# duanyiqun/DiffusionDepth

Hardware: AMD Instinct MI355X
Metric: depth-maps/sec (20-step DDIM, KITTI 352x1216 f16r, B=4 maps per GPU per step; depth RMSE vs the reference's CPU path <= 1e-3 on this workload AND at KITTI's depth range 0-80 m: see cpu_baseline.rmse_gate) (higher is better)
Workload: dtype f16 (f16 MFMA operands, fp32 accumulation; refined mode: f16-pair weights in conv1 / conv4 / conv3(cond), block-scaled int16 hand-over of y3 and conv3(cond)); 1 GPU; kitti 352x1216 image -> latent 16x176x608, cond 256x176x608, Res head denoiser (mmbev_res50 config), T=20, encoder+loop+decoder, inputs resident in HBM; global_batch=4, parallelism=dp1 (independent images, no collective), ranks_seen=1, streams=2, graph=True, variant=res

## Files before the change

### diffusiondepth_amd/csrc/dd_api.cpp

```cpp
#include "dd_api_internal.h"
#include <cstdlib>

namespace ddapi {
thread_local std::string g_create_error;
}


extern "C" {

const char* dd_version(void) { return "ddepth 0.1 gfx950 (hip, mfma bf16/f16/f32 implicit-GEMM conv3x3+GN+ReLU, hipGraph DDIM loop)"; }

const char* dd_last_error(dd_handle_t h) { return h ? h->err.c_str() : g_create_error.c_str(); }

int dd_create(dd_handle_t* out, int device, int variant) {
  if (!out) { g_create_error = "dd_create: out is NULL"; return DD_ERR_INVALID_ARG; }
  *out = nullptr;
  if (variant != DD_VARIANT_RES && variant != DD_VARIANT_SWIN) { g_create_error = "dd_create: unknown variant"; return DD_ERR_INVALID_ARG; }
  int n = 0;
  hipError_t e = hipGetDeviceCount(&n);
  if (e != hipSuccess || n <= 0) {
    g_create_error = std::string("dd_create: no HIP device available (") + (e != hipSuccess ? hipGetErrorString(e) : "count = 0") +
                     "); this library has no CPU fallback";
    return DD_ERR_HIP;
  }
// ... 94 lines not shown
    h->bf16_pure = value != 0;
  }
  else if (k == "naive_wgrad") h->naive_wgrad = value != 0;
  else if (k == "lane_probe") h->lane_probe = value != 0;
  else if (k == "x3_grad_fp32") h->x3_grad_fp32 = value != 0;
  else if (k == "keep_trajectory") h->keep_traj = value != 0;
  else if (k == "use_trajectory") h->use_traj = value;
  else if (k == "adjoint_tiled") h->adjoint_tiled = value != 0;
  else if (k == "streams") h->n_streams = value < 1 ? 1 : (int)value;
  else if (k == "keep_activations_mb") h->keep_act_mb = value < 0 ? 0 : value;
  else if (k == "big_tiles") {
    if (value < -1 || value > 1) return h->fail(DD_ERR_INVALID_ARG, "dd_set_option: big_tiles must be -1 (automatic), 0 or 1");
    if (h->big_tiles != (int)value) { DD_HIP(hipDeviceSynchronize()); h->plans.clear(); h->last_once_plan = nullptr; }
    h->big_tiles = (int)value;
  }
  else if (k == "thin_slots") {
    if (value < 1 || value > 4096) return h->fail(DD_ERR_INVALID_ARG, "dd_set_option: thin_slots must be in [1, 4096]");
    if (h->thin_slots != (int)value) { DD_HIP(hipDeviceSynchronize()); h->plans.clear(); h->last_once_plan = nullptr; }
    h->thin_slots = (int)value;
  }
  else if (k == "one_buffer") {
    if (value < 0 || value > 2) return h->fail(DD_ERR_INVALID_ARG, "dd_set_option: one_buffer must be 0, 1 or 2");
    if (h->one_buffer != (int)value) { DD_HIP(hipDeviceSynchronize()); h->plans.clear(); h->last_once_plan = nullptr; }
    h->one_buffer = (int)value;
  }
  else if (k == "cond_direct") {
    if (value < 0 || value > 1) return h->fail(DD_ERR_INVALID_ARG, "dd_set_option: cond_direct must be 0 or 1");
    h->cond_direct = (int)value;
  }
  else if (k == "cond_split") {
    if (value < 0 || value > 1) return h->fail(DD_ERR_INVALID_ARG, "dd_set_option: cond_split must be 0 or 1");
    h->cond_split = (int)value;
  }
  else if (k == "thin_stream") {
    if (value < 0 || value > 1) return h->fail(DD_ERR_INVALID_ARG, "dd_set_option: thin_stream must be 0 or 1");
    if (h->thin_stream != (int)value) {
      DD_HIP(hipDeviceSynchronize());
      h->plans.clear(); h->last_once_plan = nullptr;
    }
    h->thin_stream = (int)value;
  }
  else if (k == "f16r_wide" || k == "f16r_p4" || k == "f16r_c1") {
    if (value < 0 || value > 1) return h->fail(DD_ERR_INVALID_ARG, "dd_set_option: " + k + " must be 0 or 1");
    int& opt = k == "f16r_wide" ? h->f16r_wide : k == "f16r_c1" ? h->f16r_c1 : h->f16r_p4;
    if (opt != (int)value) { DD_HIP(hipDeviceSynchronize()); h->plans.clear(); h->last_once_plan = nullptr; }
    opt = (int)value;
  }
  else if (k == "phase_prof_buffer") h->prof_buf = reinterpret_cast<unsigned long long*>((uintptr_t)value);
  else if (k == "phase_prof_layer") h->prof_layer = (int)value;
  else if (k == "layer_timing") {
    drain_layer_events(h);
    h->layer_timing = value != 0;
    for (int i = 0; i < dd_handle_s::N_LAYER_SLOTS; ++i) { h->layer_ms[i] = 0; h->layer_cnt[i] = 0; }
  } else return h->fail(DD_ERR_INVALID_ARG, "dd_set_option: unknown key '" + k + "'");
  return DD_OK;
}

int dd_get_counter(dd_handle_t h, const char* key, int64_t* value) {
  if (!h || !key || !value) return DD_ERR_INVALID_ARG;
  const std::string k(key);
  if (k == "graph_launches") *value = h->n_graph_launches;
  else if (k == "graph_default") *value = h->graph_off_by_env ? 0 : 1;
  else if (k == "eager_loops") *value = h->n_eager_loops;
  else if (k == "graph_capture_failures") *value = h->n_capture_failures;
  else if (k == "plans") *value = (int64_t)h->plans.size();
  else if (k == "neck_launches") *value = h->n_neck_launches;
  else if (k == "trajectory_ticket") *value = h->traj_serial;
  else if (k == "lane_calls") *value = h->n_lane_calls;
  else if (k == "lane_probe_retries") *value = h->n_lane_probe_retries;
  else if (k == "lane_overlap") *value = h->lane_overlap_seen;
  else if (k == "cond_split_ok") *value = (h->fpn_committed && h->fpn_split_ok ? 1 : 0) | (h->neck_committed && h->neck_split_ok ? 2 : 0);
  else if (k == "resident_slots") *value = h->resident_slots;
  else if (k == "trajectory_reuses") *value = h->n_traj_reuse;
  else return h->fail(DD_ERR_INVALID_ARG, "dd_get_counter: unknown key '" + k + "'");
  return DD_OK;
}

// ... 457 lines not shown
  }
  h->last_once_plan = pl;
  pl->traj_ticket = (h->keep_traj && precision != DD_PREC_NAIVE_FP32) ? ++h->traj_serial : 0;
  pl->traj_weights = h->weights_serial;
  if (h->debug_sync) DD_HIP(hipStreamSynchronize(s));
  return DD_OK;
}

int dd_add_noise(dd_handle_t h, const float* x0, const float* noise, const int64_t* t, float* out, int B, int C,
                 int lat_h, int lat_w, void* stream) {
  if (!h) return DD_ERR_INVALID_ARG;
  if (h->n_train <= 0) return h->fail(DD_ERR_STATE, "schedule not set (dd_set_schedule)");
  if (!x0 || !noise || !t || !out || B <= 0 || C <= 0 || lat_h <= 0 || lat_w <= 0)
    return h->fail(DD_ERR_INVALID_ARG, "dd_add_noise: null pointer or non-positive size");
  DD_HIP(hipSetDevice(h->device));
  DD_HIP(launch_add_noise(x0, noise, reinterpret_cast<const long long*>(t), h->d_acp.as<float>(), h->n_train, out, B,
                          (long long)C * lat_h * lat_w, reinterpret_cast<hipStream_t>(stream)));
  return DD_OK;
}

static int ensure_codec_tmp(dd_handle_t h, size_t bytes) {
  if (h->codec_tmp.bytes >= bytes) return DD_OK;
  DD_HIP(hipDeviceSynchronize());
  DD_HIP(h->codec_tmp.alloc(bytes));
  return DD_OK;
}

int dd_encode(dd_handle_t h, const float* depth, float* latent, int B, int H, int W, void* stream) {
  if (!h) return DD_ERR_INVALID_ARG;
  if (!h->codec_committed) return h->fail(DD_ERR_STATE, "depth_transform.* weights not committed");
  if (!depth || !latent || B <= 0 || H <= 0 || W <= 0) return h->fail(DD_ERR_INVALID_ARG, "dd_encode: null pointer or non-positive size");
  DD_HIP(hipSetDevice(h->device));
  const int lh = (H - 1) / 2 + 1, lw = (W - 1) / 2 + 1;
  int rc = ensure_codec_tmp(h, (size_t)B * lh * lw * LATENT_C * 4);
  if (rc) return rc;
  DD_HIP(launch_encode(h->codec, depth, h->codec_tmp.as<float>(), latent, B, H, W, reinterpret_cast<hipStream_t>(stream)));
  return DD_OK;
}

int dd_decode(dd_handle_t h, const float* latent, float* depth, int B, int lat_h, int lat_w, void* stream) {
  if (!h) return DD_ERR_INVALID_ARG;
  if (!h->codec_committed) return h->fail(DD_ERR_STATE, "depth_transform.* weights not committed");
  if (!latent || !depth || B <= 0 || lat_h <= 0 || lat_w <= 0) return h->fail(DD_ERR_INVALID_ARG, "dd_decode: null pointer or non-positive size");
  DD_HIP(hipSetDevice(h->device));
  int rc = ensure_codec_tmp(h, (size_t)B * (2 * lat_h) * (2 * lat_w) * LATENT_C * 4);
  if (rc) return rc;
  DD_HIP(launch_decode(h->codec, latent, h->codec_tmp.as<float>(), depth, B, lat_h, lat_w, reinterpret_cast<hipStream_t>(stream)));
  return DD_OK;
}

int dd_debug_fetch(dd_handle_t h, const char* name, float* out, int64_t numel, void* stream) {
  if (!h || !name || !out) return DD_ERR_INVALID_ARG;
  Plan* pl = h->last_once_plan;
  if (!pl) return h->fail(DD_ERR_STATE, "dd_debug_fetch: no dd_denoise_once call to inspect");
  const std::string n(name);
  const void* src = nullptr; int C = 0; int ek = store_kind(pl->ek);
  if (n == "y1") { src = pl->y1.p; C = HID_C; }
  else if (n == "y2") { src = pl->y2.p; C = COND_C; }
  else if (n == "y3") {
    src = pl->y3.p; C = HID_C;
    if (pl->ek == EK_F16R && pl->wide) return h->fail(DD_ERR_UNSUPPORTED, "dd_debug_fetch: y3 travels as scaled int16 in this plan (option f16r_wide = 1)");
  }
  else if (n == "y4") { src = pl->y4.p; C = LATENT_C; ek = EK_F32; }
  else return h->fail(DD_ERR_INVALID_ARG, "dd_debug_fetch: unknown tensor '" + n + "'");
  if (numel != (int64_t)pl->key.B * C * pl->key.h * pl->key.w) return h->fail(DD_ERR_INVALID_ARG, "dd_debug_fetch: numel mismatch");
  DD_HIP(launch_nhwc_to_nchw_f32(src, ek, out, pl->key.B, C, pl->key.h, pl->key.w, pl->key.prec != DD_PREC_NAIVE_FP32,
// ... 42 lines not shown
```

### diffusiondepth_amd/csrc/dd_api_internal.h

```cpp
#pragma once
#include "../../include/ddepth.h"
#include "dd_kernels.h"

#include <cmath>
#include <cstdio>
#include <cstring>
#include <map>
#include <memory>
#include <set>
#include <string>
#include <tuple>
#include <vector>

using namespace dd;

namespace ddapi {

extern thread_local std::string g_create_error;

struct DevBuf {
  void* p = nullptr;
  size_t bytes = 0;
  DevBuf() = default;
  DevBuf(const DevBuf&) = delete;
// ... 73 lines not shown
  int B, h, w, ch, cw, T, prec, hoist;
  int keep = 0;
  int lane = 0;
  int lanes = 1;
  bool operator<(const PlanKey& o) const {
    return std::tie(B, h, w, ch, cw, T, prec, hoist, keep, lane, lanes) < std::tie(o.B, o.h, o.w, o.ch, o.cw, o.T, o.prec, o.hoist, o.keep, o.lane, o.lanes);
  }
};

struct Plan {
  PlanKey key{};
  int ek = EK_F32;
  DevBuf x[2];
  std::shared_ptr<DevBuf> cond;
  const void* cond_alias = nullptr;
  const void* graph_cond = nullptr;
  void* cond_ptr() const { return cond_alias ? const_cast<void*>(cond_alias) : (cond ? cond->p : nullptr); }
  DevBuf y1, y2, y3, y4;
  DevBuf a1, f, a3, eps;
  DevBuf sa, sf;
  DevBuf bX, bA1, bF, bA3;
  DevBuf bSa, bSf;
  DevBuf xstash;
  int64_t traj_ticket = 0;
  int64_t traj_weights = -1;
  bool traj_consumed = false;
  DevBuf gA, gY;
  DevBuf dgb;
  DevBuf bcorr;
  DevBuf ttab, tt_scratch;
  int64_t ttab_weights = -1;
  DevBuf ccond;
  DevBuf ccond_raw;
  DevBuf ccond_scale;
  DevBuf y3_scale;
  bool wide = false, c1 = false, p4 = false;
  DevBuf stats;
  DevBuf c1c2;
  DevBuf tsteps;
  std::vector<long long> tsteps_host;
  size_t stats_bytes = 0;
  hipGraphExec_t exec = nullptr;
  bool capture_failed = false;
  uint64_t last_use = 0;
  ~Plan() { if (exec) (void)hipGraphExecDestroy(exec); }
  int slots = 1;
  size_t kept_bytes = 0;
  void* slot(const DevBuf& b, int step) const { return static_cast<char*>(b.p) + (slots > 1 ? (size_t)step * (b.bytes / slots) : 0); }
  double* stat_ptr(int step, int layer) const {
    return stats.as<double>() + ((size_t)(step * 4 + layer) * key.B) * STAT_SLOTS * STAT_STRIDE;
  }
};

struct FpnWork {
  int B = 0, ek = -1, pyr = 0, hs[FPN_LEVELS] = {0}, ws[FPN_LEVELS] = {0};
  DevBuf fin[FPN_LEVELS];
  DevBuf lat[FPN_LEVELS];
  DevBuf up[FPN_LEVELS - 1];
  DevBuf pooled[FPN_LEVELS - 1];
  bool neck = false;
  DevBuf nk_cat[FPN_LEVELS];
  DevBuf nk_out[FPN_LEVELS];
};


struct NeckConv { int layer; std::string name; int cout, cin, ks, level, kind, C, Ck; };
// ... 63 lines not shown
  int f16r_wide = 1;
  int f16r_c1 = 1;
  int f16r_p4 = 0;
  bool split_ok = true;
  DevBuf wmax;
  int resident_slots = 512;
  hipStream_t lane_stream[MAX_LANES] = {nullptr, nullptr, nullptr, nullptr};
  std::vector<hipEvent_t> probe_events;
  std::vector<hipStream_t> burnt_streams;
  int lane_probe = 1;
  int64_t n_lane_probe_retries = 0, lane_overlap_seen = -1;
  hipEvent_t lane_fork = nullptr, lane_done[MAX_LANES] = {nullptr, nullptr, nullptr, nullptr};
  int64_t n_lane_calls = 0;
  int active_lanes = 1;
  bool adjoint_tiled = true;
  int64_t traj_serial = 0, use_traj = 0, weights_serial = 0, n_traj_reuse = 0;
  int naive_wgrad = 0;
  int x3_grad_fp32 = 0;
  std::map<PlanKey, std::unique_ptr<Plan>> plans;
  DevBuf wgrad_ws[MAX_LANES];
  std::map<std::string, std::unique_ptr<DevBuf>> grads[MAX_LANES];
  std::map<std::tuple<int, int, int, int, int>, std::pair<std::shared_ptr<DevBuf>, uint64_t>> cond_bufs;
  bool neck_committed = false;
  DevBuf neck_w[12][NUM_WIMG], neck_b[12];
  int64_t n_neck_launches = 0;
  bool fpn_committed = false;
  int fpn_pyramid = PYR_DEFAULT;
  DevBuf fpn_lat_w[FPN_LEVELS][NUM_WIMG], fpn_lat_b[FPN_LEVELS];
  DevBuf fpn_up_w[FPN_LEVELS - 1][NUM_WIMG], fpn_up_b[FPN_LEVELS - 1];
  std::unique_ptr<FpnWork> fpn_work;
  std::shared_ptr<DevBuf> fpn_out;
  bool fpn_split_ok = false, neck_split_ok = false;
  int cond_direct = 1;
  int cond_split = 1;
  std::shared_ptr<DevBuf> fpn_cond;
  int fpn_cond_key[4] = {0, 0, 0, -1};
  uint64_t tick = 0;
  Plan* last_once_plan = nullptr;
  hipEvent_t ev0 = nullptr, ev1 = nullptr;
  bool ev_valid = false;
  hipStream_t cap_stream = nullptr;
  int64_t n_graph_launches = 0, n_eager_loops = 0, n_capture_failures = 0;
  static constexpr int N_LAYER_SLOTS = 72;
  double layer_ms[N_LAYER_SLOTS] = {0};
  int64_t layer_cnt[N_LAYER_SLOTS] = {0};
  std::vector<std::tuple<int, hipEvent_t, hipEvent_t>> pending_ev;

  int fail(int code, const std::string& m) { err = m; return code; }
};

#define DD_HIP(expr)                                                                              \
  do {                                                                                            \
    hipError_t _e = (expr);                                                                       \
    if (_e != hipSuccess)                                                                         \
      return h->fail(DD_ERR_HIP, std::string(#expr) + ": " + hipGetErrorString(_e));              \
  } while (0)

namespace ddapi {
struct WeightSpec { std::string name; int64_t numel; };

inline const char* const kConvNames[4] = {"model.noise_embedding.0", "model.noise_embedding.3", "model.pred.0", "model.pred.3"};
inline const char* const kGnNames[4] = {"model.noise_embedding.1", "model.noise_embedding.4", "model.pred.1", "model.pred.4"};
constexpr int kCins[4] = {LATENT_C, HID_C, COND_C, HID_C}, kCouts[4] = {HID_C, COND_C, HID_C, LATENT_C};

int weight_group(const std::string& name);
std::vector<WeightSpec> required_weights(int variant, int pyr = PYR_DEFAULT);
// ... 36 lines not shown
```

### diffusiondepth_amd/csrc/dd_api_plans.cpp

```cpp
#include "dd_api_internal.h"

namespace ddapi {

int check_common(dd_handle_t h, int B, int lh, int lw, int ch, int cw, bool need_schedule) {
  if (!h) return DD_ERR_INVALID_ARG;
  if (!h->committed) return h->fail(DD_ERR_STATE, "model.* weights not committed (call dd_set_weight for every key, then dd_commit_weights)");
  if (need_schedule && h->n_train <= 0) return h->fail(DD_ERR_STATE, "schedule not set (dd_set_schedule)");
  if (B <= 0 || lh <= 0 || lw <= 0) return h->fail(DD_ERR_INVALID_ARG, "B, lat_h, lat_w must be positive");
  if (h->variant == DD_VARIANT_RES && (ch != lh || cw != lw))
    return h->fail(DD_ERR_INVALID_ARG, "DD_VARIANT_RES needs cond_h,cond_w == lat_h,lat_w (reference ...res.py:340 adds them elementwise)");
  if (h->variant == DD_VARIANT_SWIN && (ch <= 0 || cw <= 0)) return h->fail(DD_ERR_INVALID_ARG, "cond_h, cond_w must be positive");
  if ((long long)B * lh * lw * COND_C >= (1LL << 31) * 4) return h->fail(DD_ERR_INVALID_ARG, "tensor too large");
  return DD_OK;
}

int lane_count(dd_handle_t h, int B, int precision) {
  int S = h->n_streams;
  if (S > B) S = B;
  if (S > dd_handle_s::MAX_LANES) S = dd_handle_s::MAX_LANES;
  if (precision == DD_PREC_NAIVE_FP32 || h->layer_timing || h->debug_sync || h->prof_buf || h->check_finite) S = 1;
  return S < 1 ? 1 : S;
}

int check_split(dd_handle_t h, int precision, const char* who) {
// ... 90 lines not shown
    }
    if (victim == h->plans.end()) break;
    if (h->last_once_plan == victim->second.get()) h->last_once_plan = nullptr;
    DD_HIP(hipDeviceSynchronize());
    h->plans.erase(victim);
  }
  std::unique_ptr<Plan> pl(new Plan());
  pl->key = key;
  const bool naive = key.prec == DD_PREC_NAIVE_FP32;
  pl->ek = naive ? EK_F32 : ek_of_precision(key.prec, h->bf16_pure);
  if (pl->ek == EK_F16R && !key.hoist)
    return h->fail(DD_ERR_UNSUPPORTED, "DD_PREC_F16R runs the hoisted forward-only plans: for the Swin / MPViT denoiser those exist with option swin_w5 = 1 "
                                       "(dd_denoise / dd_denoise_trace / dd_denoise_once); training plans: DD_PREC_F16");
  const size_t px = (size_t)key.B * key.h * key.w;
  const size_t es = ek_size(pl->ek);
  DD_HIP(pl->x[0].alloc(px * LATENT_C * 4));
  DD_HIP(pl->x[1].alloc(px * LATENT_C * 4));
  if (key.keep) DD_HIP(pl->xstash.alloc((size_t)(key.T > 0 ? key.T : 1) * px * LATENT_C * 4));
  const bool swin = h->variant == DD_VARIANT_SWIN;
  (void)swin;
  if (!(pl->ek == EK_F16R && !swin && key.hoist)) { int rc = get_cond_buf(h, key.B, key.h, key.w, key.prec, &pl->cond, key.lane); if (rc) return rc; }
  pl->slots = (key.keep == 2 && key.T > 0) ? key.T : 1;
  const size_t ns = (size_t)pl->slots;
  if (swin) {
    const size_t es_s = pl->ek == EK_F16R ? 4 : es;
    DD_HIP(pl->sa.alloc(ns * px * COND_C * es_s)); DD_HIP(pl->sf.alloc(ns * px * COND_C * es_s));
  }
  if (key.hoist)
  {
    const int th = conv_pack_geom2(conv3h_kid(h, key), pl->ek).th;
    DD_HIP(pl->ccond.alloc((size_t)key.B * ((key.h + th - 1) / th) * ((key.w + 31) / 32) * th * 32 * HID_C * 4));
    if (pl->ek == EK_F16R) {
      pl->wide = h->f16r_wide != 0; pl->c1 = h->f16r_c1 != 0; pl->p4 = h->f16r_p4 != 0;
      DD_HIP(pl->ccond_raw.alloc((size_t)key.B * ((key.h + 7) / 8) * ((key.w + 31) / 32) * 8 * 32 * HID_C * 4));
      if (pl->wide) DD_HIP(pl->ccond_scale.alloc((size_t)key.B * ((key.h + th - 1) / th) * ((key.w + 31) / 32) * 4 * 2 * (th / 4) * 4));
    }
  }
  if (key.hoist && swin) {
    const int T1 = key.T > 0 ? key.T : key.B;
    const int RH = key.h < SWIN_TT_AX ? key.h : SWIN_TT_AX, RW = key.w < SWIN_TT_AX ? key.w : SWIN_TT_AX;
    DD_HIP(pl->ttab.alloc((size_t)T1 * SWIN_TT_ROWS * HID_C * 4));
    DD_HIP(pl->tt_scratch.alloc((size_t)T1 * RH * RW * (2 * COND_C + HID_C) * 4));
    if (h->swin_w5) {
      DD_HIP(pl->bcorr.alloc((size_t)key.B * swin_ring_stride(key.h, key.w) * HID_C * 4));
      DD_HIP(hipMemsetAsync(pl->bcorr.p, 0, pl->bcorr.bytes, nullptr));
      DD_HIP(hipStreamSynchronize(nullptr));
    }
  }
  DD_HIP(pl->y1.alloc(ns * px * HID_C * es));
  DD_HIP(pl->y2.alloc(ns * px * COND_C * es));
  DD_HIP(pl->y3.alloc(ns * px * HID_C * es));
  if (pl->ek == EK_F16R && h->f16r_wide) DD_HIP(pl->y3_scale.alloc(ns * px * 4));
  DD_HIP(pl->y4.alloc(ns * px * LATENT_C * 4));
  if (key.keep == 2) pl->kept_bytes = pl->y1.bytes + pl->y2.bytes + pl->y3.bytes + pl->y3_scale.bytes + pl->y4.bytes + pl->sa.bytes + pl->sf.bytes;
  if (naive) {
    DD_HIP(pl->a1.alloc(px * HID_C * 4));
    DD_HIP(pl->f.alloc(px * COND_C * 4));
    DD_HIP(pl->a3.alloc(px * HID_C * 4));
    DD_HIP(pl->eps.alloc(px * LATENT_C * 4));
  }
  const int T = key.T > 0 ? key.T : 1;
  pl->stats_bytes = (size_t)(T + 1) * 4 * key.B * STAT_SLOTS * STAT_STRIDE * sizeof(double);
  DD_HIP(pl->stats.alloc(pl->stats_bytes));
  std::vector<float> c1c2((size_t)T * 2, 0.f);
  std::vector<long long> ts((size_t)T, 0);
  if (key.T > 0) {
    const int ratio = h->n_train / key.T;
    for (int k = 0; k < key.T; ++k) {
// ... 122 lines not shown
  const PlanKey& k = pl->key;
  const int B = k.B, hh = k.h, ww = k.w;
  auto L = h->L;
  DD_HIP(launch_naive_conv3x3(x_in, L[0].w_oihw.as<float>(), L[0].bias.as<float>(), pl->y1.as<float>(), B, hh, ww, LATENT_C, HID_C, s));
  DD_HIP(launch_naive_gn_stats(pl->y1.as<float>(), pl->stat_ptr(step, 0), B, hh, ww, HID_C, s));
  DD_HIP(launch_naive_gn_apply(pl->y1.as<float>(), pl->stat_ptr(step, 0), L[0].gamma.as<float>(), L[0].beta.as<float>(),
                               nullptr, nullptr, nullptr, 0, 0, pl->a1.as<float>(), B, hh, ww, HID_C, s));
  DD_HIP(launch_naive_conv3x3(pl->a1.as<float>(), L[1].w_oihw.as<float>(), L[1].bias.as<float>(), pl->y2.as<float>(), B, hh, ww, HID_C, COND_C, s));
  DD_HIP(launch_naive_gn_stats(pl->y2.as<float>(), pl->stat_ptr(step, 1), B, hh, ww, COND_C, s));
  DD_HIP(launch_naive_gn_apply(pl->y2.as<float>(), pl->stat_ptr(step, 1), L[1].gamma.as<float>(), L[1].beta.as<float>(),
                               static_cast<const float*>(pl->cond_ptr()), h->emb.as<float>(), tvec, t_base, t_bstride, pl->f.as<float>(), B, hh, ww, COND_C, s));
  DD_HIP(launch_naive_conv3x3(pl->f.as<float>(), L[2].w_oihw.as<float>(), L[2].bias.as<float>(), pl->y3.as<float>(), B, hh, ww, COND_C, HID_C, s));
  DD_HIP(launch_naive_gn_stats(pl->y3.as<float>(), pl->stat_ptr(step, 2), B, hh, ww, HID_C, s));
  DD_HIP(launch_naive_gn_apply(pl->y3.as<float>(), pl->stat_ptr(step, 2), L[2].gamma.as<float>(), L[2].beta.as<float>(),
                               nullptr, nullptr, nullptr, 0, 0, pl->a3.as<float>(), B, hh, ww, HID_C, s));
  DD_HIP(launch_naive_conv3x3(pl->a3.as<float>(), L[3].w_oihw.as<float>(), L[3].bias.as<float>(), pl->y4.as<float>(), B, hh, ww, HID_C, LATENT_C, s));
  DD_HIP(launch_naive_gn_stats(pl->y4.as<float>(), pl->stat_ptr(step, 3), B, hh, ww, LATENT_C, s));
  DD_HIP(launch_naive_gn_apply(pl->y4.as<float>(), pl->stat_ptr(step, 3), L[3].gamma.as<float>(), L[3].beta.as<float>(),
                               nullptr, nullptr, nullptr, 0, 0, pl->eps.as<float>(), B, hh, ww, LATENT_C, s));
  if (h->debug_sync) DD_HIP(hipStreamSynchronize(s));
  return DD_OK;
}

int enqueue_cond_conv(dd_handle_t h, Plan* pl, hipStream_t s, const float* nchw) {
  const PlanKey& k = pl->key;
  ConvParams p{};
  p.B = k.B; p.h = k.h; p.w = k.w;
  p.tiles_x = (k.w + 31) / 32;
  p.ablate = 0;
  if (pl->ek == EK_F16R) {
    p.tiles_y = (k.h + 7) / 8;
    p.in = nchw ? static_cast<const void*>(nchw) : pl->cond_ptr(); p.wpack = h->L[2].wpack2[WIMG_SPLIT].p; p.bias = h->zero_bias.as<float>();
    p.out = pl->ccond_raw.p;
    DD_HIP(launch_conv_igemm2(nchw ? CONV3C_NCHW : 8, EK_F16S, p, s));
    DD_HIP(launch_cadd_reformat(pl->ccond_raw.as<float>(), pl->ccond.p, pl->ccond_scale.as<float>(), k.B, k.h, k.w, plan_big_tiles(h, k) ? 1 : 0, pl->wide ? 2 : 1, s));
    return DD_OK;
  }
  const int kid = conv3c_kid(h, k);
  p.tiles_y = (k.h + conv_pack_geom2(kid, pl->ek).th - 1) / conv_pack_geom2(kid, pl->ek).th;
  p.in = pl->cond_ptr(); p.wpack = h->L[2].wpack2[wimg_slot(thin_kind(pl->ek))].p; p.bias = h->zero_bias.as<float>(); p.out = pl->ccond.p;
  DD_HIP(launch_conv_igemm2(kid, pl->ek, p, s));
  return DD_OK;
}


int ensure_swin_w5(dd_handle_t h, hipStream_t s) {
  if (h->w5_weights == h->weights_serial) return DD_OK;
  if (!h->LB.w_oihw.p || !h->L[2].w_oihw.p) return h->fail(DD_ERR_STATE, "hoisted Swin form: the fp32 weights of convB / pred.0 are not on the device");
  if (!h->w5_oihw.p) {
    DD_HIP(h->w5_oihw.alloc((size_t)HID_C * COND_C * 25 * 4)); DD_HIP(h->pairp.alloc((size_t)81 * COND_C * HID_C * 4)); DD_HIP(h->kside.alloc(SWIN_KSIDE_BYTES));
  }
  DD_HIP(launch_swin_compose(h->LB.w_oihw.as<float>(), h->L[2].w_oihw.as<float>(), h->w5_oihw.as<float>(), h->pairp.as<float>(), h->kside.p, s));
  for (int wi = 0; wi < NUM_WIMG; ++wi) {
    if (wi == WIMG_STACK) continue;
    const int ekk = wimg_kind(wi);
    const PackGeom g5 = conv_pack_geom2(SWIN_PRED5_H, ekk);
    int rc = ensure_bytes(h, h->w5pack[wi], pack_weights_bytes(g5, ekk)); if (rc) return rc;
    DD_HIP(launch_pack_weights(h->w5_oihw.as<float>(), h->w5pack[wi].p, g5, ekk, true, false, s));
  }
  h->w5_weights = h->weights_serial;
  return DD_OK;
}

int enqueue_swin_hoist(dd_handle_t h, Plan* pl, hipStream_t s) {
  const PlanKey& k = pl->key;
  if (k.T > 0 && pl->ttab_weights != h->weights_serial) {
    if (!h->LA.w_oihw.p || !h->LB.w_oihw.p || !h->L[2].w_oihw.p) return h->fail(DD_ERR_STATE, "hoisted Swin form: the fp32 weights of the fuse convolutions are not on the device");
    DD_HIP(launch_swin_ttab(h->LA.w_oihw.as<float>(), h->LB.w_oihw.as<float>(), h->L[2].w_oihw.as<float>(), h->emb.as<float>(),
                            pl->tsteps.as<long long>(), k.T, k.h, k.w, pl->tt_scratch.as<float>(), pl->ttab.as<float>(), s));
    pl->ttab_weights = h->weights_serial;
  }
  if (pl->bcorr.p) { int rc = ensure_swin_w5(h, s); if (rc) return rc; }
  ConvParams p{};
  p.B = k.B; p.h = k.h; p.w = k.w;
  p.tiles_x = (k.w + 31) / 32;
  if (pl->ek == EK_F16R) {
    p.tiles_y = (k.h + 7) / 8;
    p.in = pl->cond_ptr(); p.wpack = h->LA.wpack2[WIMG_SPLIT].p; p.bias = h->LA.bias.as<float>(); p.out = pl->sa.p;
    DD_HIP(launch_conv_igemm2(6, EK_F16S, p, s));
    p.in = pl->sa.p; p.wpack = h->LB.wpack2[WIMG_SPLIT].p; p.bias = h->LB.bias.as<float>(); p.out = pl->sf.p;
    DD_HIP(launch_conv_igemm2(6, EK_F16S, p, s));
    p.in = pl->sf.p; p.wpack = h->L[2].wpack2[WIMG_SPLIT].p; p.bias = h->zero_bias.as<float>(); p.out = pl->ccond_raw.p;
    DD_HIP(launch_conv_igemm2(8, EK_F16S, p, s));
    DD_HIP(launch_cadd_reformat(pl->ccond_raw.as<float>(), pl->ccond.p, pl->ccond_scale.as<float>(), k.B, k.h, k.w, plan_big_tiles(h, k) ? 1 : 0, pl->wide ? 2 : 1, s));
    return DD_OK;
  }
  const int tk = thin_kind(pl->ek);
  p.tiles_y = (k.h + conv_pack_geom2(6, tk).th - 1) / conv_pack_geom2(6, tk).th;
  p.in = pl->cond_ptr(); p.wpack = h->LA.wpack2[wimg_slot(tk)].p; p.bias = h->LA.bias.as<float>(); p.out = pl->sa.p;
  DD_HIP(launch_conv_igemm2(6, tk, p, s));
  p.in = pl->sa.p; p.wpack = h->LB.wpack2[wimg_slot(tk)].p; p.bias = h->LB.bias.as<float>(); p.out = pl->sf.p;
  DD_HIP(launch_conv_igemm2(6, tk, p, s));
  const int kid8 = conv3c_kid(h, k);
  p.tiles_y = (k.h + conv_pack_geom2(kid8, pl->ek).th - 1) / conv_pack_geom2(kid8, pl->ek).th;
  p.in = pl->sf.p; p.wpack = h->L[2].wpack2[wimg_slot(tk)].p; p.bias = h->zero_bias.as<float>(); p.out = pl->ccond.p;
  DD_HIP(launch_conv_igemm2(kid8, pl->ek, p, s));
  return DD_OK;
}

int stage_condition(dd_handle_t h, Plan* pl, const float* cond, int B, int lat_h, int lat_w, int cond_h, int cond_w,
                    int precision, hipStream_t s, int img0, int whole_B) {
  if (whole_B <= 0) whole_B = B;
  pl->cond_alias = nullptr;
  const bool direct = cond && h->cond_direct && h->variant != DD_VARIANT_SWIN && pl->ek == EK_F16R && pl->key.hoist;
  if (direct) return enqueue_cond_conv(h, pl, s, cond);
  if (!pl->cond) { int rc = get_cond_buf(h, pl->key.B, pl->key.h, pl->key.w, pl->key.prec, &pl->cond, pl->key.lane); if (rc) return rc; }
  if (cond) {
    if (h->variant == DD_VARIANT_SWIN) DD_HIP(launch_upsample_to_blocked(cond, pl->cond->p, cond_kind(pl->ek), B, COND_C, cond_h, cond_w, lat_h, lat_w, s));
    else DD_HIP(launch_nchw_to_nhwc(cond, pl->cond->p, cond_kind(pl->ek), B, COND_C, cond_h, cond_w, precision != DD_PREC_NAIVE_FP32, s));
    if (h->fpn_cond == pl->cond) { h->fpn_cond.reset(); h->fpn_cond_key[3] = -1; }
  } else if (h->variant == DD_VARIANT_SWIN) {
    const int* k = h->fpn_cond_key;
    if (!h->fpn_cond || h->fpn_cond != h->fpn_out || k[0] != whole_B || k[1] != cond_h || k[2] != cond_w || k[3] != precision)
      return h->fail(DD_ERR_STATE, "cond == NULL needs a preceding dd_condition with the same batch, condition size and precision");
    const char* src = static_cast<const char*>(h->fpn_out->p) + (size_t)img0 * COND_C * cond_h * cond_w * ek_size(cond_kind(pl->ek));
// ... 49 lines not shown
```

### diffusiondepth_amd/csrc/dd_igemm2.hip

```cpp
#include "dd_igemm2_cfg.h"
#include "dd_gcn.h"

namespace dd {

#if DD_PHASE_PROF && !defined(DD_HOST_EMULATION)
#define DD_PROF_MARK(i) do { if (p.prof != nullptr && threadIdx.x == 0) p.prof[(size_t)blockIdx.x * 8 + (i)] = (unsigned long long)wall_clock64(); } while (0)
#define DD_PROF_HWID() do { if (p.prof != nullptr && threadIdx.x == 0) {                                                     \
    unsigned hw_, xcc_; asm volatile("s_getreg_b32 %0, hwreg(HW_REG_HW_ID)" : "=s"(hw_)); asm volatile("s_getreg_b32 %0, hwreg(HW_REG_XCC_ID)" : "=s"(xcc_));   \
    p.prof[(size_t)blockIdx.x * 8 + 6] = hw_; p.prof[(size_t)blockIdx.x * 8 + 7] = xcc_; } } while (0)
#define DD_PROF_CLK() ((unsigned long long)__builtin_amdgcn_s_memtime())
#define DD_PROF_LOOP_DECL unsigned long long pl_acc_[4] = {0, 0, 0, 0}, pl_t_ = 0
#define DD_PROF_LOOP_START() do { if (p.prof != nullptr) pl_t_ = DD_PROF_CLK(); } while (0)
#define DD_PROF_LOOP_ADD(k) do { if (p.prof != nullptr) { const unsigned long long n_ = DD_PROF_CLK(); pl_acc_[k] += n_ - pl_t_; pl_t_ = n_; } } while (0)
#define DD_PROF_LOOP_STORE() do { if (p.prof != nullptr && lane == 0) { for (int k_ = 0; k_ < 4; ++k_)                          \
    p.prof[(size_t)gridDim.x * 8 + ((size_t)blockIdx.x * C::WAVES + wave) * 4 + k_] = pl_acc_[k_]; } } while (0)
#else
#define DD_PROF_MARK(i) ((void)0)
#define DD_PROF_HWID() ((void)0)
#define DD_PROF_LOOP_DECL
#define DD_PROF_LOOP_START() ((void)0)
#define DD_PROF_LOOP_ADD(k) ((void)0)
#define DD_PROF_LOOP_STORE() ((void)0)
#endif

// ... 629 lines not shown
        for (int q = 0; q < 4; ++q) {
          float v[4];
          value_of(n, q, v);
          if (pvalid) {
            const float s = (v[0] + v[1]) + (v[2] + v[3]);
            const float sq = fmaf(v[0], v[0], fmaf(v[1], v[1], fmaf(v[2], v[2], v[3] * v[3])));
            const int lg = 2 * n + (q >> 1);
            ls[lg] += s; lq[lg] += sq;
          }
          pmax = fmaxf(pmax, fmaxf(fmaxf(fabsf(v[0]), fabsf(v[1])), fmaxf(fabsf(v[2]), fabsf(v[3]))));
#pragma unroll
          for (int i = 0; i < 4; ++i) acc[n][m][q * 4 + i] = v[i];
        }
      pmax = fmaxf(pmax, __shfl_xor(pmax, 32, 64));
      const float inv = pmax > 0.f ? 1.f / pmax : 0.f;
      if (pvalid && g == 0) p.out_scale[(size_t)e_b * h * w + (size_t)gy * w + gx] = pmax * (1.f / Q15_ONE);
#pragma unroll
      for (int n = 0; n < C::WN; ++n) {
        uint2 pk[4];
#pragma unroll
        for (int q = 0; q < 4; ++q) {
          pk[q].x = DD_CVT_PKNORM_I16(acc[n][m][q * 4 + 0] * inv, acc[n][m][q * 4 + 1] * inv);
          pk[q].y = DD_CVT_PKNORM_I16(acc[n][m][q * 4 + 2] * inv, acc[n][m][q * 4 + 3] * inv);
        }
#pragma unroll
        for (int k = 0; k < 2; ++k) {
          const auto rx = __builtin_amdgcn_permlane32_swap(pk[2 * k].x, pk[2 * k + 1].x, false, false);
          const auto ry = __builtin_amdgcn_permlane32_swap(pk[2 * k].y, pk[2 * k + 1].y, false, false);
          const int co = n0 + n * 32 + 16 * k + 8 * g;
          if (pvalid) *reinterpret_cast<uint4*>(out_b + act_offset(C::COUT, h, w, 0, co, gy, gx) * 2) = make_uint4(rx[0], ry[0], rx[1], ry[1]);
        }
      }
      continue;
    }
#pragma unroll
    for (int n = 0; n < C::WN; ++n) {
      uint2 pk[4];
#pragma unroll
      for (int q = 0; q < 4; ++q) {
        if (C::COUT < 32 && q >= 2) continue;
        const int co = n0 + n * 32 + 8 * q + 4 * g;
        float v[4];
        value_of(n, q, v);
        if (C::STATS && pvalid) {
          const float s = (v[0] + v[1]) + (v[2] + v[3]);
          const float sq = fmaf(v[0], v[0], fmaf(v[1], v[1], fmaf(v[2], v[2], v[3] * v[3])));
          const int lg = (C::COUT == COND_C) ? (n >> 1) : (C::COUT == HID_C) ? (2 * n + (q >> 1)) : q;
          ls[lg] += s; lq[lg] += sq;
        }
        if constexpr (C::LAYER == 8) {
          const size_t fi = ((((size_t)e_tile * C::WAVES + wave) * C::WN + n) * C::WM + m) * 256 + q * 64 + lane;
          if constexpr (C::CADD16) reinterpret_cast<uint2*>(p.out)[fi] = make_uint2(pack2<EK_F16>(v[0], v[1]), pack2<EK_F16>(v[2], v[3]));
          else reinterpret_cast<float4*>(p.out)[fi] = make_float4(v[0], v[1], v[2], v[3]);
        } else if constexpr (C::OUT_ESZ == 4) {
          if (pvalid && (C::COUT_PAD == C::COUT || co < C::COUT)) {
            if constexpr (C::SCATTER) {
              const int par = co >> 8, cc = co & (COND_C - 1);
              *reinterpret_cast<float4*>(reinterpret_cast<char*>(p.out) + ((size_t)e_b * 4 * h * w * COND_C +
                  act_offset(COND_C, 2 * h, 2 * w, 0, cc, 2 * gy + (par >> 1), 2 * gx + (par & 1))) * 4) = make_float4(v[0], v[1], v[2], v[3]);
            } else {
              *reinterpret_cast<float4*>(out_b + act_offset(C::COUT, h, w, 0, co, gy, gx) * 4) = make_float4(v[0], v[1], v[2], v[3]);
            }
          }
        } else {
          pk[q].x = pack2<C::OUT_K>(v[0], v[1]);
          pk[q].y = pack2<C::OUT_K>(v[2], v[3]);
// ... 306 lines not shown
```

### diffusiondepth_amd/csrc/dd_kernels.h

```cpp
#pragma once
#include <hip/hip_runtime.h>
#include <stdint.h>

namespace dd {

constexpr int LATENT_C = 16;
constexpr int HID_C = 64;
constexpr int COND_C = 256;
constexpr int GN_GROUPS = 4;
constexpr int EMB_ROWS = 1280;
__host__ __device__ inline long long clamp_t(long long t) { return t < 0 ? 0 : (t >= EMB_ROWS ? EMB_ROWS - 1 : t); }
constexpr float GN_EPS = 1e-5f;
constexpr float BN_EPS = 1e-5f;

constexpr int STAT_SLOTS = 32;
constexpr int STAT_STRIDE = 16;

enum ElemKind : int { EK_F32 = 0, EK_BF16 = 1, EK_F16 = 2, EK_BF16M = 3, EK_F16S = 4, EK_F16R = 5 };
constexpr float Q15_ONE = 32767.f;
__host__ __device__ constexpr int opnd_kind(int ek) { return ek == EK_BF16M ? (int)EK_BF16 : (ek == EK_F16S || ek == EK_F16R) ? (int)EK_F16 : ek; }
__host__ __device__ constexpr int store_kind(int ek) { return (ek == EK_BF16M || ek == EK_F16R) ? (int)EK_F16 : ek == EK_F16S ? (int)EK_F32 : ek; }
__host__ __device__ constexpr int cond_kind(int ek) { return ek == EK_F16R ? (int)EK_F32 : store_kind(ek); }
constexpr float STACK_LSCALE = 2048.f;
constexpr float SPLIT_WSCALE = 256.f;
// ... 1 lines not shown
__host__ __device__ constexpr float split_pscale(int pro) { return (pro == 1  || pro == 2 ) ? SPLIT_PSCALE : 1.f; }
__host__ __device__ constexpr float split_oscale(int pro) { return 1.f / (SPLIT_WSCALE * split_pscale(pro)); }

enum Prologue : int {
  PRO_X = 0,
  PRO_GN = 1,
  PRO_GN_ADD = 2,
  PRO_RAW = 3
};

struct ConvParams {
  const void* in;
  const void* wpack;
  const float* bias;
  void* out;
  double* stats_out;
  const double* stats_in;
  const float* gn_gamma;
  const float* gn_beta;
  const void* cond;
  const float* emb;
  const long long* tvec;
  int t_base, t_bstride;
  long long t_known = -1;
  const float* y4;
  float* xout;
  const float* c1c2;
  int step;
  int B, h, w;
  int tiles_x, tiles_y;
  const float* cadd;
  const float* cadd_scale;
  float* out_scale;
  const float* etab;
  const float* ttab;
  int ttab_bstride;
  const float* bcorr;
  const void* addend;
  int in_cstride, in_coff, out_cstride, out_coff;
  unsigned long long* prof;
  int persist_slots;
  int ablate;
};

constexpr int BIG_CONV3C = 48, BIG_CONV3H = 49;
constexpr int ONE_CONV3H = 46;
constexpr int CONV3C_NCHW = 47;
constexpr int SWIN_CONVA_H = 50, SWIN_PRED_H = 52;
constexpr int SWIN_PRED5_H = 53;
constexpr int SWIN_PRED5B_H = 51;
__host__ __device__ inline int swin_ring_size(int h, int w) { return 2 * w + 2 * (h > 2 ? h - 2 : 0); }
__host__ __device__ inline int swin_ring_stride(int h, int w) { return swin_ring_size(h, w) + 4; }
__host__ __device__ inline int swin_ring_index(int y, int x, int h, int w) {
  return y == 0 ? x : (y == h - 1 ? w + x : (x == 0 ? 2 * w + (y - 1) : 2 * w + (h - 2) + (y - 1)));
}
constexpr int SWIN_TT_AX = 7, SWIN_TT_ROWS = 1 + SWIN_TT_AX * SWIN_TT_AX;
__host__ __device__ inline int swin_tt_class(int y, int n) { const int R = n < SWIN_TT_AX ? n : SWIN_TT_AX; return y < 3 ? y : (y >= n - 3 ? R - (n - y) : 3); }
__host__ __device__ inline int swin_tt_ref(int n) { return n - 1 < 3 ? n - 1 : 3; }
inline int persist_grid(int B, int tiles_per_img, int slots) {
  int n = slots / (B > 0 ? B : 1);
  if (n < 1) n = 1;
  if (n > tiles_per_img) n = tiles_per_img;
  return B * n;
}
struct PackGeom { int cin, cout, cout_pad, ck, tg, nt, th, ks, planes, stack; };
hipError_t launch_conv_igemm2(int layer, int ek, const ConvParams& p, hipStream_t s);
// ... 82 lines not shown
```

### diffusiondepth_amd/csrc/dd_misc.hip

```cpp
#include "dd_elem.h"
#include "dd_gcn.h"

namespace dd {
__device__ __forceinline__ float relu_keep_nan(float v) { return (v < 0.f) ? 0.f : v; }


__device__ __forceinline__ uint32_t cvt_bf16(float f) {
  uint32_t u = __builtin_bit_cast(uint32_t, f);
  u += 0x7FFFu + ((u >> 16) & 1u);
  return u >> 16;
}
__device__ __forceinline__ uint32_t cvt_f16(float f) { return (uint32_t)__builtin_bit_cast(uint16_t, (_Float16)f); }
__device__ __forceinline__ float ld_elem(const void* base, size_t idx, int ek) {
  if (ek == EK_F32) return reinterpret_cast<const float*>(base)[idx];
  const uint32_t u = reinterpret_cast<const uint16_t*>(base)[idx];
  return ek == EK_BF16 ? __builtin_bit_cast(float, u << 16) : (float)__builtin_bit_cast(_Float16, (uint16_t)u);
}

template <int EK>
__global__ void __launch_bounds__(256) nchw_to_nhwc_kernel(const float* __restrict__ src, void* __restrict__ dst,
                                                           int C, int Cd, long long HW, int blocked) {
  __shared__ float tile[64][65];
  const int b = blockIdx.z;
  const long long p0 = (long long)blockIdx.x * 64;
// ... 724 lines not shown
  };
  fetch(0, cur, cur_in);
#pragma unroll 1
  for (int tap = 0; tap < 9; ++tap) {
    fetch(tap < 8 ? tap + 1 : 8, nx, nx_in);
    float in[LATENT_C];
#pragma unroll
    for (int q = 0; q < 4; ++q) {
      in[4 * q] = cur_in ? cur[q].x : 0.f; in[4 * q + 1] = cur_in ? cur[q].y : 0.f; in[4 * q + 2] = cur_in ? cur[q].z : 0.f; in[4 * q + 3] = cur_in ? cur[q].w : 0.f;
    }
    const float* wt = w1t + (size_t)tap * LATENT_C * LATENT_C;
#pragma unroll
    for (int q = 0; q < LATENT_C / 4; ++q) {
#pragma unroll
      for (int j = 0; j < 4; ++j) {
        const int ci = 4 * q + j;
        const f32x2_t* row = reinterpret_cast<const f32x2_t*>(wt + ci * LATENT_C);
        const f32x2_t a = (f32x2_t){in[ci], in[ci]};
#pragma unroll
        for (int co = 0; co < LATENT_C / 2; ++co) acc[co] = __builtin_elementwise_fma(row[co], a, acc[co]);
      }
      DD_SCHED_FENCE();
    }
#pragma unroll
    for (int q = 0; q < 4; ++q) cur[q] = nx[q];
    cur_in = nx_in;
  }
  if (ok) {
#pragma unroll
    for (int c = 0; c < LATENT_C; ++c) latent[((size_t)b * LATENT_C + c) * HW + p] = tanhf(acc[c >> 1][c & 1]);
  }
}

hipError_t launch_encode(const CodecWeights& cw, const float* depth, float* tmp_nhwc, float* latent_nchw,
                         int B, int H, int W, hipStream_t s) {
  const int h = (H - 1) / 2 + 1, w = (W - 1) / 2 + 1;
  dim3 grid((unsigned)(((long long)h * w + 255) / 256), (unsigned)B);
  hipLaunchKernelGGL(enc0_kernel, grid, dim3(256), 0, s, depth, cw.enc_w0, cw.enc_b0, tmp_nhwc, H, W, h, w);
  hipLaunchKernelGGL(enc1_kernel, grid, dim3(256), 0, s, tmp_nhwc, cw.enc_w1t, cw.enc_b1, latent_nchw, h, w);
  return hipGetLastError();
}

__global__ void __launch_bounds__(256) dec0_kernel(const float* __restrict__ latent, const float* __restrict__ w0,
                                                   const float* __restrict__ b0, float* __restrict__ tmp, int h, int w) {
  const int b = blockIdx.y;
  const int H = 2 * h, W = 2 * w;
  const long long HW = (long long)h * w;
  const long long p = (long long)blockIdx.x * blockDim.x + threadIdx.x;
  if (p >= (long long)H * W) return;
  const int oy = (int)(p / W), ox = (int)(p - (long long)oy * W);
  float acc[LATENT_C];
#pragma unroll
  for (int c = 0; c < LATENT_C; ++c) acc[c] = b0[c];
  const float* lat = latent + (size_t)b * LATENT_C * HW;
#pragma unroll
  for (int a = 0; a < 2; ++a) {
    const int ky = ((oy + 1) & 1) + 2 * a;
    const int iy = (oy + 1 - ky) >> 1;
    if (iy < 0 || iy >= h) continue;
#pragma unroll
    for (int c2 = 0; c2 < 2; ++c2) {
      const int kx = ((ox + 1) & 1) + 2 * c2;
      const int ix = (ox + 1 - kx) >> 1;
      if (ix < 0 || ix >= w) continue;
      for (int ci = 0; ci < LATENT_C; ++ci) {
        const float v = lat[(size_t)ci * HW + (size_t)iy * w + ix];
        const float* wr = w0 + ((size_t)ci * LATENT_C) * 16 + ky * 4 + kx;
#pragma unroll
        for (int co = 0; co < LATENT_C; ++co) acc[co] = fmaf(wr[co * 16], v, acc[co]);
// ... 295 lines not shown
```

Before: 557.7 maps/s.

## Fuse cond-add reformat into conv3 epilogue and fuse encoder conv pair

The conv3(cond) split-f16 igemm epilogue now writes directly in the tiled cond-add layout, either f16 or block-scaled int16 with a per-block max scale. This removes the fp32 ccond_raw buffer and the separate launch_cadd_reformat pass. Separately, the depth encoder's two convolutions are fused into one kernel that recomputes the first layer with a halo in shared memory, avoiding the NHWC temp round-trip. Both paths are on by default; the risk is extra halo recompute, and zero-padding the ccond buffers when tile heights disagree.

```diff
diff --git a/diffusiondepth_amd/csrc/dd_api.cpp b/diffusiondepth_amd/csrc/dd_api.cpp
--- a/diffusiondepth_amd/csrc/dd_api.cpp
+++ b/diffusiondepth_amd/csrc/dd_api.cpp
@@ -150,6 +150,10 @@
     if (value < 0 || value > 1) return h->fail(DD_ERR_INVALID_ARG, "dd_set_option: cond_split must be 0 or 1");
     h->cond_split = (int)value;
   }
+  else if (k == "enc_fused") {
+    if (value < 0 || value > 1) return h->fail(DD_ERR_INVALID_ARG, "dd_set_option: enc_fused must be 0 or 1");
+    h->enc_fused = (int)value;
+  }
   else if (k == "thin_stream") {
     if (value < 0 || value > 1) return h->fail(DD_ERR_INVALID_ARG, "dd_set_option: thin_stream must be 0 or 1");
     if (h->thin_stream != (int)value) {
@@ -158,9 +162,9 @@
     }
     h->thin_stream = (int)value;
   }
-  else if (k == "f16r_wide" || k == "f16r_p4" || k == "f16r_c1") {
+  else if (k == "f16r_wide" || k == "f16r_p4" || k == "f16r_c1" || k == "cadd_fused") {
     if (value < 0 || value > 1) return h->fail(DD_ERR_INVALID_ARG, "dd_set_option: " + k + " must be 0 or 1");
-    int& opt = k == "f16r_wide" ? h->f16r_wide : k == "f16r_c1" ? h->f16r_c1 : h->f16r_p4;
+    int& opt = k == "f16r_wide" ? h->f16r_wide : k == "f16r_c1" ? h->f16r_c1 : k == "cadd_fused" ? h->cadd_fused : h->f16r_p4;
     if (opt != (int)value) { DD_HIP(hipDeviceSynchronize()); h->plans.clear(); h->last_once_plan = nullptr; }
     opt = (int)value;
   }
@@ -684,6 +688,10 @@
   if (!depth || !latent || B <= 0 || H <= 0 || W <= 0) return h->fail(DD_ERR_INVALID_ARG, "dd_encode: null pointer or non-positive size");
   DD_HIP(hipSetDevice(h->device));
   const int lh = (H - 1) / 2 + 1, lw = (W - 1) / 2 + 1;
+  if (h->enc_fused) {
+    DD_HIP(launch_encode(h->codec, depth, nullptr, latent, B, H, W, reinterpret_cast<hipStream_t>(stream)));
+    return DD_OK;
+  }
   int rc = ensure_codec_tmp(h, (size_t)B * lh * lw * LATENT_C * 4);
   if (rc) return rc;
   DD_HIP(launch_encode(h->codec, depth, h->codec_tmp.as<float>(), latent, B, H, W, reinterpret_cast<hipStream_t>(stream)));
diff --git a/diffusiondepth_amd/csrc/dd_api_internal.h b/diffusiondepth_amd/csrc/dd_api_internal.h
--- a/diffusiondepth_amd/csrc/dd_api_internal.h
+++ b/diffusiondepth_amd/csrc/dd_api_internal.h
@@ -129,6 +129,7 @@
   int64_t ttab_weights = -1;
   DevBuf ccond;
   DevBuf ccond_raw;
+  bool cfused = false;
   DevBuf ccond_scale;
   DevBuf y3_scale;
   bool wide = false, c1 = false, p4 = false;
@@ -258,6 +259,8 @@
   std::shared_ptr<DevBuf> fpn_out;
   bool fpn_split_ok = false, neck_split_ok = false;
   int cond_direct = 1;
+  int cadd_fused = 1;
+  int enc_fused = 1;
   int cond_split = 1;
   std::shared_ptr<DevBuf> fpn_cond;
   int fpn_cond_key[4] = {0, 0, 0, -1};
diff --git a/diffusiondepth_amd/csrc/dd_api_plans.cpp b/diffusiondepth_amd/csrc/dd_api_plans.cpp
--- a/diffusiondepth_amd/csrc/dd_api_plans.cpp
+++ b/diffusiondepth_amd/csrc/dd_api_plans.cpp
@@ -146,8 +146,14 @@
     DD_HIP(pl->ccond.alloc((size_t)key.B * ((key.h + th - 1) / th) * ((key.w + 31) / 32) * th * 32 * HID_C * 4));
     if (pl->ek == EK_F16R) {
       pl->wide = h->f16r_wide != 0; pl->c1 = h->f16r_c1 != 0; pl->p4 = h->f16r_p4 != 0;
-      DD_HIP(pl->ccond_raw.alloc((size_t)key.B * ((key.h + 7) / 8) * ((key.w + 31) / 32) * 8 * 32 * HID_C * 4));
+      pl->cfused = h->cadd_fused != 0;
+      if (!pl->cfused) DD_HIP(pl->ccond_raw.alloc((size_t)key.B * ((key.h + 7) / 8) * ((key.w + 31) / 32) * 8 * 32 * HID_C * 4));
       if (pl->wide) DD_HIP(pl->ccond_scale.alloc((size_t)key.B * ((key.h + th - 1) / th) * ((key.w + 31) / 32) * 4 * 2 * (th / 4) * 4));
+      if (pl->cfused && th == 16 && ((key.h + 15) / 16) * 16 != ((key.h + 7) / 8) * 8) {
+        DD_HIP(hipMemsetAsync(pl->ccond.p, 0, pl->ccond.bytes, nullptr));
+        if (pl->wide) DD_HIP(hipMemsetAsync(pl->ccond_scale.p, 0, pl->ccond_scale.bytes, nullptr));
+        DD_HIP(hipStreamSynchronize(nullptr));
+      }
     }
   }
   if (key.hoist && swin) {
@@ -336,6 +342,11 @@
     p.tiles_y = (k.h + 7) / 8;
     p.in = nchw ? static_cast<const void*>(nchw) : pl->cond_ptr(); p.wpack = h->L[2].wpack2[WIMG_SPLIT].p; p.bias = h->zero_bias.as<float>();
     p.out = pl->ccond_raw.p;
+    if (pl->cfused) {
+      p.out = pl->ccond.p; p.out_scale = pl->ccond_scale.as<float>(); p.cadd_kind = pl->wide ? 2 : 1; p.cadd_big = plan_big_tiles(h, k) ? 1 : 0;
+      DD_HIP(launch_conv_igemm2(nchw ? CONV3C_NCHW : 8, EK_F16S, p, s));
+      return DD_OK;
+    }
     DD_HIP(launch_conv_igemm2(nchw ? CONV3C_NCHW : 8, EK_F16S, p, s));
     DD_HIP(launch_cadd_reformat(pl->ccond_raw.as<float>(), pl->ccond.p, pl->ccond_scale.as<float>(), k.B, k.h, k.w, plan_big_tiles(h, k) ? 1 : 0, pl->wide ? 2 : 1, s));
     return DD_OK;
@@ -385,6 +396,11 @@
     p.in = pl->sa.p; p.wpack = h->LB.wpack2[WIMG_SPLIT].p; p.bias = h->LB.bias.as<float>(); p.out = pl->sf.p;
     DD_HIP(launch_conv_igemm2(6, EK_F16S, p, s));
     p.in = pl->sf.p; p.wpack = h->L[2].wpack2[WIMG_SPLIT].p; p.bias = h->zero_bias.as<float>(); p.out = pl->ccond_raw.p;
+    if (pl->cfused) {
+      p.out = pl->ccond.p; p.out_scale = pl->ccond_scale.as<float>(); p.cadd_kind = pl->wide ? 2 : 1; p.cadd_big = plan_big_tiles(h, k) ? 1 : 0;
+      DD_HIP(launch_conv_igemm2(8, EK_F16S, p, s));
+      return DD_OK;
+    }
     DD_HIP(launch_conv_igemm2(8, EK_F16S, p, s));
     DD_HIP(launch_cadd_reformat(pl->ccond_raw.as<float>(), pl->ccond.p, pl->ccond_scale.as<float>(), k.B, k.h, k.w, plan_big_tiles(h, k) ? 1 : 0, pl->wide ? 2 : 1, s));
     return DD_OK;
diff --git a/diffusiondepth_amd/csrc/dd_igemm2.hip b/diffusiondepth_amd/csrc/dd_igemm2.hip
--- a/diffusiondepth_amd/csrc/dd_igemm2.hip
+++ b/diffusiondepth_amd/csrc/dd_igemm2.hip
@@ -685,6 +685,42 @@
         }
       }
       continue;
+    }
+    if constexpr (C::LAYER == 8 && C::SPLIT) {
+      if (p.cadd_kind != 0) {
+        static_assert(C::WM == 2 && C::WN == 2 && C::WAVES == 4, "block order of the 8x32 split-f16 tiles");
+        size_t blk0; int nstride;
+        if (p.cadd_big) {
+          const int y = e_y0 + wave * C::WM + m;
+          const size_t tile2 = ((size_t)e_b * ((h + 15) >> 4) + (y >> 4)) * p.tiles_x + (e_x0 >> 5);
+          blk0 = ((tile2 * 4 + ((y & 15) >> 2)) * 2) * 4 + (y & 3); nstride = 4;
+        } else { blk0 = (((size_t)e_tile * 4 + wave) * 2) * 2 + m; nstride = 2; }
+#pragma unroll
+        for (int n = 0; n < C::WN; ++n) {
+          float v[4][4];
+#pragma unroll
+          for (int q = 0; q < 4; ++q) value_of(n, q, v[q]);
+          const size_t blk = blk0 + (size_t)n * nstride;
+          uint2* dst = reinterpret_cast<uint2*>(p.out) + blk * 256 + lane;
+          if (p.cadd_kind == 2) {
+            auto nmax = [](float a, float b) { return (b > a || b != b) ? b : a; };
+            float mx = 0.f;
+#pragma unroll
+            for (int q = 0; q < 4; ++q) mx = nmax(mx, nmax(nmax(fabsf(v[q][0]), fabsf(v[q][1])), nmax(fabsf(v[q][2]), fabsf(v[q][3]))));
+#pragma unroll
+            for (int off = 32; off >= 1; off >>= 1) mx = nmax(mx, __shfl_xor(mx, off, 64));
+            const float inv = mx > 0.f ? 1.f / mx : 0.f;
+            if (lane == 0) p.out_scale[blk] = mx * (1.f / Q15_ONE);
+#pragma unroll
+            for (int q = 0; q < 4; ++q)
+              dst[q * 64] = make_uint2(DD_CVT_PKNORM_I16(v[q][0] * inv, v[q][1] * inv), DD_CVT_PKNORM_I16(v[q][2] * inv, v[q][3] * inv));
+          } else {
+#pragma unroll
+            for (int q = 0; q < 4; ++q) dst[q * 64] = make_uint2(pack2<EK_F16>(v[q][0], v[q][1]), pack2<EK_F16>(v[q][2], v[q][3]));
+          }
+        }
+        continue;
+      }
     }
 #pragma unroll
     for (int n = 0; n < C::WN; ++n) {
diff --git a/diffusiondepth_amd/csrc/dd_kernels.h b/diffusiondepth_amd/csrc/dd_kernels.h
--- a/diffusiondepth_amd/csrc/dd_kernels.h
+++ b/diffusiondepth_amd/csrc/dd_kernels.h
@@ -57,6 +57,7 @@
   const float* cadd;
   const float* cadd_scale;
   float* out_scale;
+  int cadd_kind = 0, cadd_big = 0;
   const float* etab;
   const float* ttab;
   int ttab_bstride;
diff --git a/diffusiondepth_amd/csrc/dd_misc.hip b/diffusiondepth_amd/csrc/dd_misc.hip
--- a/diffusiondepth_amd/csrc/dd_misc.hip
+++ b/diffusiondepth_amd/csrc/dd_misc.hip
@@ -780,9 +780,93 @@
   }
 }
 
+constexpr int ET_H = 8, ET_W = 32;
+constexpr int ER_H = ET_H + 2, ER_W = ET_W + 2;
+constexpr int ER_P = LATENT_C + 4;
+static_assert(ET_H * ET_W == 256, "one latent pixel per work-item");
+__global__ void __launch_bounds__(256) enc_fused_kernel(const float* __restrict__ depth, const float* __restrict__ w0, const float* __restrict__ b0,
+                                                        const float* __restrict__ w1t, const float* __restrict__ b1, float* __restrict__ latent,
+                                                        int H, int W, int h, int w) {
+  __shared__ __attribute__((aligned(16))) float s_mid[ER_H][ER_W][ER_P];
+  const int b = blockIdx.z;
+  const int Y0 = blockIdx.y * ET_H, X0 = blockIdx.x * ET_W;
+  const int tid = threadIdx.x;
+  const float* d = depth + (size_t)b * H * W;
+  for (int i = tid; i < ER_H * ER_W; i += 256) {
+    const int r = i / ER_W, c = i - r * ER_W;
+    const int oy = Y0 - 1 + r, ox = X0 - 1 + c;
+    const bool inside = oy >= 0 && oy < h && ox >= 0 && ox < w;
+    float in[9];
+#pragma unroll
+    for (int ky = 0; ky < 3; ++ky)
+#pragma unroll
+      for (int kx = 0; kx < 3; ++kx) {
+        const int iy = 2 * oy - 1 + ky, ix = 2 * ox - 1 + kx;
+        in[ky * 3 + kx] = (inside && iy >= 0 && iy < H && ix >= 0 && ix < W) ? d[(size_t)iy * W + ix] : 0.f;
+      }
+    float o[LATENT_C];
+#pragma unroll
+    for (int co = 0; co < LATENT_C; ++co) {
+      float a = b0[co];
+#pragma unroll
+      for (int k = 0; k < 9; ++k) a = fmaf(w0[co * 9 + k], in[k], a);
+      o[co] = inside ? (a >= 0.f ? a : 0.2f * a) : 0.f;
+    }
+    float4* dst = reinterpret_cast<float4*>(&s_mid[r][c][0]);
+#pragma unroll
+    for (int q = 0; q < 4; ++q) dst[q] = make_float4(o[4 * q], o[4 * q + 1], o[4 * q + 2], o[4 * q + 3]);
+  }
+  __syncthreads();
+  const int ty = tid / ET_W, tx = tid - ty * ET_W;
+  const int oy = Y0 + ty, ox = X0 + tx;
+  f32x2_t acc[LATENT_C / 2];
+#pragma unroll
+  for (int c = 0; c < LATENT_C / 2; ++c) acc[c] = (f32x2_t){b1[2 * c], b1[2 * c + 1]};
+  float4 cur[4], nx[4];
+  auto fetch = [&](int tap, float4 (&dst)[4]) {
+    const int ky = tap / 3, kx = tap - ky * 3;
+    const float4* src = reinterpret_cast<const float4*>(&s_mid[ty + ky][tx + kx][0]);
+#pragma unroll
+    for (int q = 0; q < 4; ++q) dst[q] = src[q];
+  };
+  fetch(0, cur);
+#pragma unroll 1
+  for (int tap = 0; tap < 9; ++tap) {
+    fetch(tap < 8 ? tap + 1 : 8, nx);
+    float in[LATENT_C];
+#pragma unroll
+    for (int q = 0; q < 4; ++q) { in[4 * q] = cur[q].x; in[4 * q + 1] = cur[q].y; in[4 * q + 2] = cur[q].z; in[4 * q + 3] = cur[q].w; }
+    const float* wt = w1t + (size_t)tap * LATENT_C * LATENT_C;
+#pragma unroll
+    for (int q = 0; q < LATENT_C / 4; ++q) {
+#pragma unroll
+      for (int j = 0; j < 4; ++j) {
+        const int ci = 4 * q + j;
+        const f32x2_t* row = reinterpret_cast<const f32x2_t*>(wt + ci * LATENT_C);
+        const f32x2_t a = (f32x2_t){in[ci], in[ci]};
+#pragma unroll
+        for (int co = 0; co < LATENT_C / 2; ++co) acc[co] = __builtin_elementwise_fma(row[co], a, acc[co]);
+      }
+      DD_SCHED_FENCE();
+    }
+#pragma unroll
+    for (int q = 0; q < 4; ++q) cur[q] = nx[q];
+  }
+  if (oy < h && ox < w) {
+    const size_t HW = (size_t)h * w;
+#pragma unroll
+    for (int c = 0; c < LATENT_C; ++c) latent[((size_t)b * LATENT_C + c) * HW + (size_t)oy * w + ox] = tanhf(acc[c >> 1][c & 1]);
+  }
+}
+
 hipError_t launch_encode(const CodecWeights& cw, const float* depth, float* tmp_nhwc, float* latent_nchw,
                          int B, int H, int W, hipStream_t s) {
   const int h = (H - 1) / 2 + 1, w = (W - 1) / 2 + 1;
+  if (tmp_nhwc == nullptr) {
+    dim3 grid((unsigned)((w + ET_W - 1) / ET_W), (unsigned)((h + ET_H - 1) / ET_H), (unsigned)B);
+    hipLaunchKernelGGL(enc_fused_kernel, grid, dim3(256), 0, s, depth, cw.enc_w0, cw.enc_b0, cw.enc_w1t, cw.enc_b1, latent_nchw, H, W, h, w);
+    return hipGetLastError();
+  }
   dim3 grid((unsigned)(((long long)h * w + 255) / 256), (unsigned)B);
   hipLaunchKernelGGL(enc0_kernel, grid, dim3(256), 0, s, depth, cw.enc_w0, cw.enc_b0, tmp_nhwc, H, W, h, w);
   hipLaunchKernelGGL(enc1_kernel, grid, dim3(256), 0, s, tmp_nhwc, cw.enc_w1t, cw.enc_b1, latent_nchw, h, w);
```

New measurement: 559.1 maps/s, median of 6. Within noise of the previous version (+0.3%).
